# ctxnn/GenConViT

Hardware: AMD Instinct MI355X
Metric: frames/sec (224x224, ed+vae forward) (higher is better)
Workload: dtype f16

## Files before the change

genconvit_amd/_lib.py:

```python
from __future__ import annotations

import ctypes
import ctypes.util
import json
import os
import threading

_HERE = os.path.dirname(os.path.abspath(__file__))
LIB_PATH = os.environ.get("GCV_LIB_PATH") or os.path.join(_HERE, "lib", "libgenconvit_hip.so")

GCV_F32, GCV_BF16, GCV_F16 = 0, 1, 2
ACT_NONE, ACT_RELU, ACT_GELU, ACT_LEAKY = 0, 1, 2, 3
A_PLAIN, A_IM2COL3_POOL, A_IM2COL3_S2 = 0, 1, 2
EPI_BIAS_ACT, EPI_RESID, EPI_POOL4, EPI_CONVT, EPI_SPLITK = 0, 1, 2, 3, 4

c_void_p, c_int, c_int64, c_float, c_char_p, c_size_t = (ctypes.c_void_p, ctypes.c_int, ctypes.c_int64,
                                                         ctypes.c_float, ctypes.c_char_p, ctypes.c_size_t)


class TensorDesc(ctypes.Structure):
    _fields_ = [("name", c_char_p), ("data", c_void_p), ("numel", c_int64), ("on_device", c_int)]


class GemmArgs(ctypes.Structure):
# ... 40 lines not shown
                                c_int, c_void_p, c_void_p]),
    "gcv_vote_segments": (c_int, [c_void_p, c_int, c_int, c_void_p, c_int, c_void_p, c_void_p]),
    "gcv_tap_set": (c_int, [c_void_p, c_char_p, c_void_p, c_size_t]),
    "gcv_tap_clear": (c_int, [c_void_p]),
    "gcv_tap_written": (c_int, [c_void_p, c_char_p]),
    "gcv_profile_enable": (c_int, [c_void_p, c_int]),
    "gcv_profile_report": (c_char_p, [c_void_p]),
    "gcv_k_gemm": (c_int, [c_int, c_int, c_int, ctypes.POINTER(GemmArgs), c_void_p]),
    "gcv_k_stem_ln": (c_int, [c_int, c_void_p, c_int64, c_int64, c_int64, c_int64, c_void_p, c_void_p, c_void_p,
                              c_void_p, c_void_p, c_int, c_int, c_int, c_float, c_void_p]),
    "gcv_k_stem_ln_c": (c_int, [c_int, c_void_p, c_int64, c_int64, c_int64, c_int64, c_void_p, c_void_p, c_void_p,
                                c_void_p, c_void_p, c_int, c_int, c_int, c_int, c_float, c_void_p]),
    "gcv_k_dwconv7_ln": (c_int, [c_int, c_void_p, c_void_p, c_void_p, c_void_p, c_void_p, c_void_p, c_int, c_int,
                                 c_int, c_int, c_float, c_void_p]),
    "gcv_dw_plan": (c_int, [c_int, c_int, c_int, c_int, c_int, c_int, c_void_p]),
    "gcv_convnext_res_ok": (c_int, [c_int, c_int]),
    "gcv_k_ln_patchify": (c_int, [c_int, c_void_p, c_void_p, c_void_p, c_void_p, c_int, c_int, c_int, c_int, c_float,
                                  c_void_p]),
    "gcv_k_layernorm_rows": (c_int, [c_int, c_void_p, c_void_p, c_void_p, c_void_p, c_int64, c_int, c_float, c_void_p]),
    "gcv_k_pool_ln": (c_int, [c_int, c_void_p, c_void_p, c_void_p, c_void_p, c_int, c_int, c_int, c_float, c_void_p]),
    "gcv_k_conv3_first": (c_int, [c_int, c_void_p, c_int64, c_int64, c_int64, c_int64, c_void_p, c_void_p, c_void_p,
                                  c_int, c_int, c_int, c_int, c_int, c_void_p]),
    "gcv_k_convt2_small": (c_int, [c_int, c_void_p, c_void_p, c_void_p, c_void_p, c_int, c_int, c_int, c_int, c_void_p]),
    "gcv_k_reparam": (c_int, [c_int, c_void_p, c_int, c_void_p, c_void_p, c_void_p, c_void_p, c_int, c_int, c_void_p]),
    "gcv_k_head_tail": (c_int, [c_int, c_void_p, c_void_p, c_void_p, c_void_p, c_int, c_int, c_void_p]),
    "gcv_k_head_tail_splitk": (c_int, [c_int, c_void_p, c_int, c_void_p, c_int, c_void_p, c_void_p, c_void_p, c_int, c_int,
                                       c_void_p]),
    "gcv_k_resize_mse": (c_int, [c_int, c_void_p, c_void_p, c_void_p, c_void_p, c_void_p, c_int, c_void_p]),
    "gcv_k_swin_window_attn": (c_int, [c_int, c_void_p, c_void_p, c_void_p, c_int, c_int, c_int, c_int, c_int, c_int,
                                       c_void_p]),
    "gcv_k_patch_merge_ln": (c_int, [c_int, c_void_p, c_void_p, c_void_p, c_void_p, c_int, c_int, c_int, c_int, c_float,
                                     c_void_p]),
    "gcv_k_mean_tokens": (c_int, [c_int, c_void_p, c_void_p, c_int, c_int, c_int, c_void_p]),
    "gcv_k_fused_mlp": (c_int, [c_int, c_int, c_void_p, c_void_p, c_void_p, c_void_p, c_void_p, c_void_p, c_void_p,
                                c_void_p, c_int, c_void_p]),
    "gcv_k_fused_mlp_lnp": (c_int, [c_int, c_int, c_void_p, c_void_p, c_void_p, c_void_p, c_void_p, c_void_p, c_void_p,
                                    c_void_p, c_void_p, c_float, c_int, c_void_p, c_void_p, c_void_p, c_void_p, c_void_p,
                                    c_int, c_void_p]),
    "gcv_k_fused_mlp_timed": (c_int, [c_int, c_int, c_void_p, c_void_p, c_void_p, c_void_p, c_void_p, c_void_p,
                                      c_void_p, c_void_p, c_int, c_int, c_void_p, c_void_p]),
}

_lib = None
_lock = threading.Lock()


# ... 493 lines not shown
```

genconvit_amd/csrc/api.hip:

```cpp
#include "../../include/genconvit_hip.h"

#include <dlfcn.h>

#include <cstdio>
#include <cstdlib>
#include <cstring>
#include <map>
#include <mutex>
#include <set>
#include <sstream>
#include <vector>

#include "cnx_mlp.h"
#include "gemm.h"
#include "kernels.h"
#include "net.h"

namespace gcv {
static thread_local std::string g_err;
void set_error(const std::string& msg) { g_err = msg; }
const char* get_error() { return g_err.c_str(); }

int ensure_dynamic_lds(const void* fn, int bytes) {
  static std::mutex mu;
  static std::map<std::pair<const void*, int>, int> done;
  int dev = 0;
  GCV_CHECK_HIP(hipGetDevice(&dev));
  std::lock_guard<std::mutex> lk(mu);
  auto it = done.find({fn, dev});
  if (it != done.end() && it->second >= bytes) return 0;
  GCV_CHECK_HIP(hipFuncSetAttribute(fn, hipFuncAttributeMaxDynamicSharedMemorySize, bytes));
  done[{fn, dev}] = bytes;
  return 0;
}

hipEvent_t Profiler::get_event() {
// ... 594 lines not shown
}

int gcv_k_layernorm_rows(int dtype, const void* x, const float* w, const float* b, void* out, int64_t rows, int C,
                         float eps, gcv_stream s) {
  DISPATCH_DT(dtype, launch_layernorm_rows<T>((const T*)x, w, b, (T*)out, rows, C, eps, (hipStream_t)s));
}

int gcv_k_pool_ln(int dtype, const void* x, const float* w, const float* b, void* out, int nimg, int HW, int C,
                  float eps, gcv_stream s) {
  DISPATCH_DT(dtype, launch_pool_ln<T>((const T*)x, w, b, (T*)out, nimg, HW, C, eps, (hipStream_t)s));
}

int gcv_k_conv3_first(int dtype, const void* x, int64_t sb, int64_t sc, int64_t sy, int64_t sx, const float* wp,
                      const float* bias, void* out, int nimg, int H, int W, int pool, int act, gcv_stream s) {
  DISPATCH_DT(dtype, launch_conv3_first<T>((const T*)x, sb, sc, sy, sx, wp, bias, (T*)out, nimg, H, W, pool != 0, act,
                                           (hipStream_t)s));
}

int gcv_k_convt2_small(int dtype, const void* x, const float* wp, const float* bias, void* out, int nimg, int H,
                       int W, int act, gcv_stream s) {
  DISPATCH_DT(dtype, launch_convt2_small<T>((const T*)x, wp, bias, (T*)out, nimg, H, W, act, (hipStream_t)s));
}

int gcv_k_reparam(int dtype, const float* partial, int splitk, const float* bias, const float* eps, float* mu_out,
                  void* z_nhwc, int B, int N, gcv_stream s) {
  DISPATCH_DT(dtype, launch_reparam<T>(partial, splitk, bias, eps, mu_out, (T*)z_nhwc, B, N, (hipStream_t)s));
}

int gcv_k_head_tail(int dtype, const void* h, const float* w, const float* bias, float* logits, int B, int K,
                    gcv_stream s) {
  DISPATCH_DT(dtype, launch_head_tail<T>((const T*)h, w, bias, logits, B, K, (hipStream_t)s));
}

int gcv_k_head_tail_splitk(int dtype, const float* partial, int splitk, const float* b1, int act, const float* w,
                           const float* bias, float* logits, int B, int K, gcv_stream s) {
  DISPATCH_DT(dtype, launch_head_tail_splitk<T>(partial, splitk, b1, act, w, bias, logits, B, K, (hipStream_t)s));
}

int gcv_k_resize_mse(int dtype, const void* xhat, const void* img, void* recon, float* msepart, float* mse, int B,
                     gcv_stream s) {
  DISPATCH_DT(dtype, launch_resize_mse<T>((const T*)xhat, (const T*)img, (T*)recon, msepart, mse, B, (hipStream_t)s));
}

int gcv_k_swin_window_attn(int dtype, const void* qkv, const float* rpb, void* out, int nimg, int H, int W, int C,
                           int nH, int shift, gcv_stream s) {
  DISPATCH_DT(dtype, launch_swin_window_attn<T>((const T*)qkv, rpb, (T*)out, nimg, H, W, C, nH, shift, (hipStream_t)s));
// ... 61 lines not shown
```

genconvit_amd/csrc/kern_bf16.hip:

```cpp
#include "kernels_impl.h"
namespace gcv { GCV_INSTANTIATE_KERNELS(bf16_t) }
```

genconvit_amd/csrc/kern_f16.hip:

```cpp
#include "kernels_impl.h"
namespace gcv { GCV_INSTANTIATE_KERNELS(half_t) }
```

genconvit_amd/csrc/net_impl.h:

```cpp
#pragma once
#include <algorithm>
#include <cmath>
#include <cstdlib>
#include <cstring>

#include "cam.h"
#include "cam_bwd.h"
#include "cnx_mlp.h"
#include "gemm.h"
#include "kernels.h"
#include "net.h"
#include "swin.h"

namespace gcv {

template <typename T> inline T host_cvt(float v);
template <> inline float host_cvt<float>(float v) { return v; }
template <> inline half_t host_cvt<half_t>(float v) { return (half_t)v; }
template <> inline bf16_t host_cvt<bf16_t>(float v) {
  uint32_t u;
  std::memcpy(&u, &v, 4);
  uint16_t h;
  if ((u & 0x7fffffffu) > 0x7f800000u) h = (uint16_t)((u >> 16) | 0x40);
  else h = (uint16_t)((u + 0x7fffu + ((u >> 16) & 1u)) >> 16);
  bf16_t r;
  std::memcpy(&r, &h, 2);
  return r;
}

struct WeightStore {
  std::vector<void*> ptrs;
// ... 60 lines not shown
  CnxMlpW<T> mlp;
};
template <typename T> struct CnxW {
  float *stem_w, *stem_b, *stem_lnw, *stem_lnb;
  CnxBlockW<T> blk[kMaxCnxBlocks];
  struct { float *ln_w, *ln_b, *b; T* w; } down[3];
  float *head_lnw, *head_lnb, *head_fc_b;
  T* head_fc_w;
  T *bwd_w1t[3], *bwd_w2t[3], *bwd_downt;
};
template <typename T> struct HeadW {
  T* fc_w;
  float* fc_b;
  float* fc2_w;
  float* fc2_b;
};
template <typename T> struct EdW {
  float *enc1_w, *enc1_b;
  T* enc_w[4];
  float* enc_b[4];
  T* dec_w[4];
  float* dec_b[4];
  float *dec5_w, *dec5_b;
  HeadW<T> head;
};
template <typename T> struct VaeW {
  float *enc1_w, *enc1_b;
  T* enc_w[3];
  float* enc_b[3];
  T *mu_w, *var_w;
  float *mu_b, *var_b;
  T* dec_w[3];
  float* dec_b[3];
  float *dec4_w, *dec4_b;
  HeadW<T> head;
};

template <typename T> struct Stage3In {
  const T* s2 = nullptr;
  const T* x[3] = {nullptr, nullptr, nullptr};
};
template <typename T> struct Seg {
  const T* x;
  int64_t sb, sc, sy, sx;
  int n, H, W;
  T* out;
  int out_ld;
  int act;
  T* pre = nullptr;
  const T** s3 = nullptr;
  Stage3In<T>* in3 = nullptr;
};

template <typename T> struct NetImpl : NetBase {
  WeightStore ws_ed, ws_vae, ws_swin;
  CnxW<T> bb_ed{}, bb_vae{};
  EdW<T> ed{};
// ... 191 lines not shown
  int up_convt_gemm(const TensorMap& w, const std::string& name, int cin, int cout, WeightStore& st, T*& dst) {
    std::vector<float> v;
    GCV_TRY(fetch(w, name, (int64_t)cin * cout * 4, v));
    std::vector<T> o((size_t)cin * cout * 4);
    for (int ci = 0; ci < cin; ++ci)
      for (int co = 0; co < cout; ++co)
        for (int dy = 0; dy < 2; ++dy)
          for (int dx = 0; dx < 2; ++dx)
            o[((size_t)(dy * 2 + dx) * cout + co) * cin + ci] = host_cvt<T>(v[(((size_t)ci * cout + co) * 2 + dy) * 2 + dx]);
    GCV_UP(dst, st, o);
    return 0;
  }
  int up_convt_small(const TensorMap& w, const std::string& name, WeightStore& st, float*& dst) {
    std::vector<float> v;
    GCV_TRY(fetch(w, name, 16 * 3 * 4, v));
    std::vector<float> o(16 * 12);
    for (int ci = 0; ci < 16; ++ci)
      for (int co = 0; co < 3; ++co)
        for (int dy = 0; dy < 2; ++dy)
          for (int dx = 0; dx < 2; ++dx) o[ci * 12 + (dy * 2 + dx) * 3 + co] = v[((ci * 3 + co) * 2 + dy) * 2 + dx];
    GCV_UP(dst, st, o);
    return 0;
  }
  int up_conv_first(const TensorMap& w, const std::string& name, const std::vector<float>* scale, WeightStore& st,
                    float*& dst) {
    std::vector<float> v;
    GCV_TRY(fetch(w, name, 16 * 27, v));
    std::vector<float> o(27 * 16);
    for (int co = 0; co < 16; ++co)
      for (int ci = 0; ci < 3; ++ci)
        for (int ky = 0; ky < 3; ++ky)
          for (int kx = 0; kx < 3; ++kx)
            o[((ky * 3 + kx) * 3 + ci) * 16 + co] = v[((co * 3 + ci) * 3 + ky) * 3 + kx] * (scale ? (*scale)[co] : 1.0f);
    GCV_UP(dst, st, o);
    return 0;
  }

  int pack_mlp(const TensorMap& w, const std::string& fc2_name, int C, WeightStore& st, CnxMlpW<T>& mw) {
    if (mw.kind == MlpKind::Gemm) return 0;
    struct DevBuf {
      float* p = nullptr;
      ~DevBuf() { if (p) (void)hipFree(p); }
    } w2f;
    if (mlp_packs_from_f32(mw.kind)) {
      std::vector<float> v;
      GCV_TRY(fetch(w, fc2_name, (int64_t)4 * C * C, v));
// ... 76 lines not shown

  int load_ed(const TensorMap& w) override {
    GCV_CHECK_HIP(hipSetDevice(device));
    has_ed = false;
    ws_ed.clear();
    GCV_TRY(up_conv_first(w, "encoder.features.0.weight", nullptr, ws_ed, ed.enc1_w));
    GCV_TRY(up_f32(w, "encoder.features.0.bias", 16, ws_ed, ed.enc1_b));
    const int ech[5] = {16, 32, 64, 128, 256};
    const int eidx[4] = {3, 6, 9, 12};
    for (int l = 0; l < 4; ++l) {
      const std::string n = "encoder.features." + std::to_string(eidx[l]);
      GCV_TRY(up_conv_gemm(w, n + ".weight", ech[l + 1], ech[l], 3, 3, nullptr, ws_ed, ed.enc_w[l]));
      GCV_TRY(up_f32(w, n + ".bias", ech[l + 1], ws_ed, ed.enc_b[l]));
    }
    const int dch[5] = {256, 128, 64, 32, 16};
    const int didx[4] = {0, 2, 4, 6};
    for (int l = 0; l < 4; ++l) {
      const std::string n = "decoder.features." + std::to_string(didx[l]);
      GCV_TRY(up_convt_gemm(w, n + ".weight", dch[l], dch[l + 1], ws_ed, ed.dec_w[l]));
      GCV_TRY(up_f32(w, n + ".bias", dch[l + 1], ws_ed, ed.dec_b[l]));
    }
    GCV_TRY(up_convt_small(w, "decoder.features.8.weight", ws_ed, ed.dec5_w));
    GCV_TRY(up_f32(w, "decoder.features.8.bias", 3, ws_ed, ed.dec5_b));
    GCV_TRY(pack_convnext(w, "backbone.", ws_ed, bb_ed));
    GCV_TRY(pack_head(w, ws_ed, ed.head));
    has_ed = true;
    return 0;
  }

  int pack_mu(const TensorMap& w, const std::string& name, T*& dst) {
    auto it = w.find(name);
    const int64_t total = (int64_t)12544 * 25088;
    if (it == w.end() || it->second.numel != total) { set_error("missing or mis-sized '" + name + "'"); return -4; }
    dst = (T*)ws_vae.raw((size_t)total * sizeof(T));
    if (!dst) { set_error("hipMalloc failed for " + name); return -5; }
    const float* src = it->second.data;
    if (it->second.on_device) {
      hipLaunchKernelGGL((pack_mu_kernel<T>), dim3((unsigned)cdiv64(total, 256)), dim3(256), 0, 0, src, dst, total);
      GCV_CHECK_HIP(hipGetLastError());
      GCV_CHECK_HIP(hipDeviceSynchronize());
      return 0;
    }
    constexpr int64_t kRows = 512;
    struct DevBuf {
      float* p = nullptr;
      ~DevBuf() { if (p) (void)hipFree(p); }
// ... 35 lines not shown
        GCV_UP(vae.enc1_b, ws_vae, bias);
      } else {
        GCV_TRY(up_conv_gemm(w, cn + ".weight", c, ech[l], 3, 3, &scale, ws_vae, vae.enc_w[l - 1]));
        GCV_UP(vae.enc_b[l - 1], ws_vae, bias);
      }
    }
    GCV_TRY(pack_mu(w, "encoder.mu.weight", vae.mu_w));
    GCV_TRY(up_f32(w, "encoder.mu.bias", 12544, ws_vae, vae.mu_b));
    vae.var_w = nullptr;
    vae.var_b = nullptr;
    if (w.count("encoder.var.weight")) {
      GCV_TRY(pack_mu(w, "encoder.var.weight", vae.var_w));
      GCV_TRY(up_f32(w, "encoder.var.bias", 12544, ws_vae, vae.var_b));
    }
    const int dch[4] = {256, 64, 32, 16};
    const int didx[3] = {0, 2, 4};
    for (int l = 0; l < 3; ++l) {
      const std::string n = "decoder.features." + std::to_string(didx[l]);
      GCV_TRY(up_convt_gemm(w, n + ".weight", dch[l], dch[l + 1], ws_vae, vae.dec_w[l]));
      GCV_TRY(up_f32(w, n + ".bias", dch[l + 1], ws_vae, vae.dec_b[l]));
    }
    GCV_TRY(up_convt_small(w, "decoder.features.6.weight", ws_vae, vae.dec4_w));
    GCV_TRY(up_f32(w, "decoder.features.6.bias", 3, ws_vae, vae.dec4_b));
    GCV_TRY(pack_convnext(w, "convnext_backbone.", ws_vae, bb_vae));
    GCV_TRY(pack_head(w, ws_vae, vae.head));
    has_vae = true;
    return 0;
  }

  int load_swin(const TensorMap& w, const std::string& prefix) override {
    GCV_CHECK_HIP(hipSetDevice(device));
    has_swin = false;
    ws_swin.clear();
    GCV_TRY((pack_swin<T>(*this, w, prefix, swin)));
    has_swin = true;
    return 0;
  }

  int run_convnext(const CnxW<T>& w, const Seg<T>* segs, int nseg, bool keep = false, const TapPass* tp = nullptr) {
    int segn[4], h[4], wd[4];
    int64_t m[4], moff[4], M = 0;
    int ntot = 0;
    GCV_REQUIRE(nseg >= 1 && nseg <= 4, "1..4 segments");
    for (int s = 0; s < nseg; ++s) {
      GCV_REQUIRE(segs[s].H % 4 == 0 && segs[s].W % 4 == 0 && segs[s].n > 0, "segment geometry");
      segn[s] = segs[s].n;
// ... 314 lines not shown
    T* rec = arena.get<T>((int64_t)B * 224 * 224 * 3);
    T* feat = arena.get<T>((int64_t)B * 2000);
    T* bbpre = ex ? arena.get<T>((int64_t)B * 2000) : nullptr;
    if (!arena.dry && arena.overflow) { set_error("workspace arena too small"); return -6; }

    GCV_TRY(run("ed.enc1_conv3_relu_pool", 2.0 * B * 224 * 224 * 16 * 27,
                sizeof(T) * (double)B * (3 * 224 * 224 + 16 * 112 * 112), [&] {
      return launch_conv3_first<T>(x, 3 * 224 * 224, 224 * 224, 224, 1, ed.enc1_w, ed.enc1_b, e1, B, 224, 224, true,
                                   ACT_RELU, cur);
    }));
    {
      const T* in[4] = {e1, e2, e3, e4};
      T* out[4] = {e2, e3, e4, e5};
      const int Hs[4] = {112, 56, 28, 14};
      const int cl[4] = {4, 5, 6, 7};
      for (int l = 0; l < 4; ++l) {
        GemmArgs g{};
        g.A = in[l]; g.Wt = ed.enc_w[l]; g.C = out[l]; g.bias = ed.enc_b[l];
        g.M = B * Hs[l] * Hs[l]; g.N = 2 << cl[l]; g.K = 9 << cl[l]; g.ldc = g.N; g.act = ACT_RELU; g.splitk = 1;
        g.H = Hs[l]; g.W = Hs[l]; g.cin_log2 = cl[l];
        GCV_TRY(gemm("ed.enc_conv3_relu_pool", g, A_IM2COL3_POOL, EPI_POOL4));
      }
    }
    {
      const T* in[4] = {e5, d1, d2, d3};
      T* out[4] = {d1, d2, d3, d4};
      const int Hs[4] = {7, 14, 28, 56};
      const int col[4] = {7, 6, 5, 4};
      for (int l = 0; l < 4; ++l) {
        GemmArgs g{};
        g.A = in[l]; g.lda = 2 << col[l]; g.Wt = ed.dec_w[l]; g.C = out[l]; g.bias = ed.dec_b[l];
        g.M = B * Hs[l] * Hs[l]; g.N = 4 << col[l]; g.K = 2 << col[l]; g.act = ACT_RELU; g.splitk = 1;
        g.H = Hs[l]; g.W = Hs[l]; g.cout_log2 = col[l];
        GCV_TRY(gemm("ed.dec_convT_relu", g, A_PLAIN, EPI_CONVT));
      }
    }
    GCV_TRY(run("ed.dec5_convT_relu", 2.0 * B * 112 * 112 * 16 * 12,
                sizeof(T) * (double)B * (16 * 112 * 112 + 3 * 224 * 224),
                [&] { return launch_convt2_small<T>(d4, ed.dec5_w, ed.dec5_b, rec, B, 112, 112, ACT_RELU, cur); }));
    Seg<T> segs[2];
    segs[0] = Seg<T>{rec, (int64_t)224 * 224 * 3, 1, 224 * 3, 3, B, 224, 224, feat, 2000, ACT_GELU};
    segs[1] = Seg<T>{x, (int64_t)3 * 224 * 224, 224 * 224, 224, 1, B, 224, 224, feat + 1000, 2000, ACT_GELU};
    const T* s3[2] = {nullptr, nullptr};
    Stage3In<T> in3[2];
    const float* head_part = nullptr;
    if (ex)
      for (int q = 0; q < 2; ++q) {
        segs[q].pre = bbpre + 1000 * q; segs[q].s3 = &s3[q];
        if (ex->layer == 2) segs[q].in3 = &in3[q];
      }
    const TapPass tp{"ed", 2, 0, {B, B}, {224, 224}, {224, 224}};
    GCV_TRY(run_convnext(bb_ed, segs, 2, false, taps.empty() ? nullptr : &tp));
    GCV_TRY(run_head(ed.head, feat, B, ACT_GELU, logits, ex ? &head_part : nullptr));
    if (ex) {
      const int hwp[2] = {49, 49}, side[2] = {7, 7}, off[2] = {0, 49}, side2[2] = {14, 14};
      GCV_TRY(explain_tail(bb_ed, ed.head, ACT_GELU, B, head_part, bbpre, logits, s3, hwp, side, off, 1, *ex, in3, side2, "ed"));
    }
    if (!taps.empty()) {
      const T* et[5] = {e1, e2, e3, e4, e5};
      const int64_t ee[5] = {112 * 112 * 16, 56 * 56 * 32, 28 * 28 * 64, 14 * 14 * 128, 7 * 7 * 256};
      const T* dt[4] = {d1, d2, d3, d4};
      const int64_t de[4] = {14 * 14 * 128, 28 * 28 * 64, 56 * 56 * 32, 112 * 112 * 16};
// ... 74 lines not shown
      for (int l = 0; l < 3; ++l) {
        GemmArgs g{};
        g.A = in[l]; g.Wt = vae.enc_w[l]; g.C = out[l]; g.bias = vae.enc_b[l];
        g.M = B * (Hs[l] / 2) * (Hs[l] / 2); g.N = 2 << cl[l]; g.K = 9 << cl[l]; g.ldc = g.N; g.act = ACT_LEAKY;
        g.splitk = 1; g.H = Hs[l]; g.W = Hs[l]; g.cin_log2 = cl[l];
        GCV_TRY(gemm("vae.enc_conv3s2_bn_leaky", g, A_IM2COL3_S2, EPI_BIAS_ACT));
      }
    }
    {
      GemmArgs g{};
      g.A = v4; g.lda = 25088; g.Wt = vae.mu_w; g.partial = part; g.M = B; g.N = 12544; g.K = 25088;
      g.splitk = SPLITK; g.k_per_split = KPS; g.act = ACT_NONE;
      GCV_TRY(gemm("vae.mu_gemm_splitk", g, A_PLAIN, EPI_SPLITK));
      GCV_TRY(run("vae.reparam", 4.0 * B * 12544, 4.0 * (SPLITK + 2) * (double)B * 12544, [&] {
        return launch_reparam<T>(part, SPLITK, vae.mu_b, eps, mu, z, B, 12544, cur);
      }));
      if (kl) {
        g.Wt = vae.var_w;
        GCV_TRY(gemm("vae.var_gemm_splitk", g, A_PLAIN, EPI_SPLITK));
        GCV_TRY(run("vae.kl", 6.0 * B * 12544, 4.0 * (SPLITK + 1) * (double)B * 12544,
                    [&] { return launch_kl(part, SPLITK, vae.var_b, mu, rowsum, kl, B, 12544, cur); }));
      }
    }
    {
      const T* in[3] = {z, d1, d2};
      T* out[3] = {d1, d2, d3};
      const int Hs[3] = {7, 14, 28};
      const int cin[3] = {256, 64, 32};
      const int col[3] = {6, 5, 4};
      for (int l = 0; l < 3; ++l) {
        GemmArgs g{};
        g.A = in[l]; g.lda = cin[l]; g.Wt = vae.dec_w[l]; g.C = out[l]; g.bias = vae.dec_b[l];
        g.M = B * Hs[l] * Hs[l]; g.N = 4 << col[l]; g.K = cin[l]; g.act = ACT_LEAKY; g.splitk = 1;
        g.H = Hs[l]; g.W = Hs[l]; g.cout_log2 = col[l];
        GCV_TRY(gemm("vae.dec_convT_leaky", g, A_PLAIN, EPI_CONVT));
      }
    }
    GCV_TRY(run("vae.dec4_convT_leaky", 2.0 * B * 56 * 56 * 16 * 12,
                sizeof(T) * (double)B * (16 * 56 * 56 + 3 * 112 * 112),
                [&] { return launch_convt2_small<T>(d3, vae.dec4_w, vae.dec4_b, xhat, B, 56, 56, ACT_LEAKY, cur); }));
    if (after_chain && !arena.dry) GCV_TRY(after_chain());
    if (split) { GCV_TRY(run_convnext(bb_vae, &segs[1], 1, true, tapping ? &tp1 : nullptr)); }
    else { GCV_TRY(run_convnext(bb_vae, segs, 2, false, tapping ? &tp0 : nullptr)); }
    join.now();
    if (tapping) {
      const T* vt[4] = {v1, v2, v3, v4};
      const int64_t ve[4] = {112 * 112 * 16, 56 * 56 * 32, 28 * 28 * 64, 14 * 14 * 128};
      const T* dt[3] = {d1, d2, d3};
      const int64_t de[3] = {14 * 14 * 64, 28 * 28 * 32, 56 * 56 * 16};
      for (int l = 0; l < 4; ++l) GCV_TRY(tap_net(("vae.v" + std::to_string(l + 1)).c_str(), vt[l], B * ve[l] * sizeof(T)));
      GCV_TRY(tap_net("vae.mu", mu, (size_t)B * 12544 * sizeof(float)));
      GCV_TRY(tap_net("vae.z", z, (size_t)B * 12544 * sizeof(T)));
      for (int l = 0; l < 3; ++l) GCV_TRY(tap_net(("vae.d" + std::to_string(l + 1)).c_str(), dt[l], B * de[l] * sizeof(T)));
      GCV_TRY(tap_net("vae.xhat", xhat, (size_t)B * 112 * 112 * 3 * sizeof(T)));
      GCV_TRY(tap_net("vae.feat", feat, (size_t)B * 2000 * sizeof(T)));
    }
    GCV_TRY(run_head(vae.head, feat, B, ACT_RELU, logits, ex ? &head_part : nullptr));
    if (ex) {
      const int hwp[2] = {49, 9}, side[2] = {7, 3}, off[2] = {0, 49}, side2[2] = {14, 7};
      GCV_TRY(explain_tail(bb_vae, vae.head, ACT_RELU, B, head_part, bbpre, logits, s3, hwp, side, off, 0, *ex, in3, side2, "vae"));
    }
    if (recon224 || mse) {
      GCV_TRY(run("vae.resize_mse", 30.0 * B * 224 * 224, sizeof(T) * (double)B * (3 * 112 * 112 + 6 * 224 * 224), [&] {
// ... 53 lines not shown
```

include/genconvit_hip.h:

```cpp
#ifndef GENCONVIT_HIP_H
#define GENCONVIT_HIP_H

#include <stddef.h>
#include <stdint.h>

#ifdef __cplusplus
extern "C" {
#endif

#if defined(GCV_BUILD)
#pragma GCC visibility push(default)
#endif

typedef struct gcv_handle gcv_handle;
typedef void* gcv_stream;

enum { GCV_F32 = 0, GCV_BF16 = 1, GCV_F16 = 2 };
enum { GCV_CONVNEXT_TINY = 0, GCV_CONVNEXT_LARGE = 1 };
enum { GCV_LARGE_MAX_BATCH = 256 };
enum { GCV_ACT_NONE = 0, GCV_ACT_RELU = 1, GCV_ACT_GELU = 2, GCV_ACT_LEAKY = 3 };

typedef struct {
  const char* name;
  const void* data;
// ... 80 lines not shown
} gcv_gemm_args;

int gcv_k_gemm(int dtype, int a_mode, int epi, const gcv_gemm_args* a, gcv_stream s);
int gcv_k_stem_ln(int dtype, const void* x, int64_t sb, int64_t sc, int64_t sy, int64_t sx, const float* wp,
                  const float* bias, const float* lnw, const float* lnb, void* out, int nimg, int Ho, int Wo,
                  float eps, gcv_stream s);
int gcv_k_stem_ln_c(int dtype, const void* x, int64_t sb, int64_t sc, int64_t sy, int64_t sx, const float* wp,
                    const float* bias, const float* lnw, const float* lnb, void* out, int nimg, int Ho, int Wo, int C,
                    float eps, gcv_stream s);
int gcv_k_dwconv7_ln(int dtype, const void* x, const float* wdw, const float* bdw, const float* lnw,
                     const float* lnb, void* y, int nimg, int H, int W, int C, float eps, gcv_stream s);
int gcv_dw_plan(int dtype, int nimg, int H, int W, int C, int aligned, int* out5);
int gcv_convnext_res_ok(int arch, int res);
int gcv_k_ln_patchify(int dtype, const void* x, const float* w, const float* b, void* out, int nimg, int H, int W,
                      int C, float eps, gcv_stream s);
int gcv_k_layernorm_rows(int dtype, const void* x, const float* w, const float* b, void* out, int64_t rows, int C,
                         float eps, gcv_stream s);
int gcv_k_pool_ln(int dtype, const void* x, const float* w, const float* b, void* out, int nimg, int HW, int C,
                  float eps, gcv_stream s);
int gcv_k_conv3_first(int dtype, const void* x, int64_t sb, int64_t sc, int64_t sy, int64_t sx, const float* wp,
                      const float* bias, void* out, int nimg, int H, int W, int pool, int act, gcv_stream s);
int gcv_k_convt2_small(int dtype, const void* x, const float* wp, const float* bias, void* out, int nimg, int H,
                       int W, int act, gcv_stream s);
int gcv_k_reparam(int dtype, const float* partial, int splitk, const float* bias, const float* eps, float* mu_out,
                  void* z_nhwc, int B, int N, gcv_stream s);
int gcv_k_head_tail(int dtype, const void* h, const float* w, const float* bias, float* logits, int B, int K,
                    gcv_stream s);
int gcv_k_head_tail_splitk(int dtype, const float* partial, int splitk, const float* b1, int act, const float* w,
                           const float* bias, float* logits, int B, int K, gcv_stream s);
int gcv_k_resize_mse(int dtype, const void* xhat, const void* img, void* recon, float* msepart, float* mse, int B,
                     gcv_stream s);

int gcv_k_swin_window_attn(int dtype, const void* qkv, const float* rpb, void* out, int nimg, int H, int W, int C,
                           int nH, int shift, gcv_stream s);
int gcv_k_patch_merge_ln(int dtype, const void* x, const float* w, const float* b, void* out, int nimg, int H, int W,
                         int C, float eps, gcv_stream s);
int gcv_k_mean_tokens(int dtype, const void* x, void* out, int nimg, int L, int C, gcv_stream s);

int gcv_k_fused_mlp(int dtype, int C, const void* x, const void* w1, const float* b1, const float* w2_f32,
                    const float* b2, const float* gamma, const void* resid, void* out, int M, gcv_stream s);
int gcv_k_fused_mlp_lnp(int dtype, int C, const void* x, const void* w1, const float* b1, const float* w2_f32,
                        const float* b2, const float* gamma, const void* resid, const float* ln_w, const float* ln_b,
                        float eps, int nseg, const int* tok0, const int* hw, const int* wd, const int* out0, void* out, int M,
                        gcv_stream s);
int gcv_k_fused_mlp_timed(int dtype, int C, const void* x, const void* w1, const float* b1, const float* w2_f32,
                          const float* b2, const float* gamma, const void* resid, void* out, int M, int iters,
// ... 11 lines not shown
```

Baseline: 18890.

## Fuse ED and VAE transposed-conv decoder chains into one LDS-resident kernel

Adds a single kernel that runs all 2x2-stride transposed-conv decoder layers plus the final small conv for each 8-pixel latent tile. Intermediates stay in shared memory, so the per-layer global round trips and separate launches go away. Layers use MFMA with weights pre-packed into fragment order at load time, and the next layer's first weight fragment is prefetched. In exchange it needs large LDS per block (two workgroups per CU) and grid parallelism is limited to B*49/8 blocks, so work per block may serialize. The fused path applies only to 16-bit types when no taps are requested.

```diff
diff --git a/genconvit_amd/_lib.py b/genconvit_amd/_lib.py
--- a/genconvit_amd/_lib.py
+++ b/genconvit_amd/_lib.py
@@ -86,6 +86,8 @@
     "gcv_k_conv3_first": (c_int, [c_int, c_void_p, c_int64, c_int64, c_int64, c_int64, c_void_p, c_void_p, c_void_p,
                                   c_int, c_int, c_int, c_int, c_int, c_void_p]),
     "gcv_k_convt2_small": (c_int, [c_int, c_void_p, c_void_p, c_void_p, c_void_p, c_int, c_int, c_int, c_int, c_void_p]),
+    "gcv_k_convt_pack": (c_int, [c_int, c_void_p, c_int, c_int, c_void_p, c_void_p]),
+    "gcv_k_decoder_fused": (c_int, [c_int, c_int, c_void_p, c_void_p, c_void_p, c_void_p, c_void_p, c_void_p, c_int, c_void_p]),
     "gcv_k_reparam": (c_int, [c_int, c_void_p, c_int, c_void_p, c_void_p, c_void_p, c_void_p, c_int, c_int, c_void_p]),
     "gcv_k_head_tail": (c_int, [c_int, c_void_p, c_void_p, c_void_p, c_void_p, c_int, c_int, c_void_p]),
     "gcv_k_head_tail_splitk": (c_int, [c_int, c_void_p, c_int, c_void_p, c_int, c_void_p, c_void_p, c_void_p, c_int, c_int,
diff --git a/genconvit_amd/csrc/api.hip b/genconvit_amd/csrc/api.hip
--- a/genconvit_amd/csrc/api.hip
+++ b/genconvit_amd/csrc/api.hip
@@ -12,6 +12,7 @@
 #include <vector>
 
 #include "cnx_mlp.h"
+#include "decoder_fused.h"
 #include "gemm.h"
 #include "kernels.h"
 #include "net.h"
@@ -652,6 +653,27 @@
   DISPATCH_DT(dtype, launch_convt2_small<T>((const T*)x, wp, bias, (T*)out, nimg, H, W, act, (hipStream_t)s));
 }
 
+int gcv_k_convt_pack(int dtype, const void* wt, int N, int K, void* dst, gcv_stream s) {
+  switch (dtype) {
+    case GCV_BF16: return launch_convt_pack<bf16_t>((const bf16_t*)wt, N, K, (bf16_t*)dst, (hipStream_t)s);
+    case GCV_F16:  return launch_convt_pack<half_t>((const half_t*)wt, N, K, (half_t*)dst, (hipStream_t)s);
+    default: set_error("convt_pack: 16-bit storage only"); return -2;
+  }
+}
+
+int gcv_k_decoder_fused(int dtype, int kind, const void* x, const void* wpk, const float* const* bias, const float* w5,
+                        const float* b5, void* out, int npix, gcv_stream s) {
+  GCV_REQUIRE(bias, "null bias list");
+  DecoderArgs a{};
+  a.x = x; a.wpk = wpk; a.w5 = w5; a.b5 = b5; a.out = out; a.npix = npix;
+  for (int l = 0; l < (kind == DEC_ED ? 4 : 3); ++l) a.bias[l] = bias[l];
+  switch (dtype) {
+    case GCV_BF16: return launch_decoder_fused<bf16_t>(kind, a, (hipStream_t)s);
+    case GCV_F16:  return launch_decoder_fused<half_t>(kind, a, (hipStream_t)s);
+    default: set_error("decoder_fused: 16-bit storage only"); return -2;
+  }
+}
+
 int gcv_k_reparam(int dtype, const float* partial, int splitk, const float* bias, const float* eps, float* mu_out,
                   void* z_nhwc, int B, int N, gcv_stream s) {
   DISPATCH_DT(dtype, launch_reparam<T>(partial, splitk, bias, eps, mu_out, (T*)z_nhwc, B, N, (hipStream_t)s));
diff --git a/genconvit_amd/csrc/decoder_fused.h b/genconvit_amd/csrc/decoder_fused.h
--- /dev/null
+++ b/genconvit_amd/csrc/decoder_fused.h
@@ -0,0 +1,302 @@
+#pragma once
+#include "common.h"
+#include "gemm.h"
+
+namespace gcv {
+
+enum { DEC_ED = 0, DEC_VAE = 1 };
+
+struct DecoderArgs {
+  const void* x;
+  const void* wpk;
+  const float* bias[4];
+  const float* w5;
+  const float* b5;
+  void* out;
+  int npix;
+};
+
+inline int64_t decoder_packed_elems(int kind) {
+  return kind == DEC_ED ? 4 * (256 * 128 + 128 * 64 + 64 * 32 + 32 * 16) : 4 * (256 * 64 + 64 * 32 + 32 * 16);
+}
+template <typename T> int launch_convt_pack(const T* wt, int N, int K, T* dst, hipStream_t s);
+template <typename T> int launch_decoder_fused(int kind, const DecoderArgs& a, hipStream_t s);
+
+#ifdef GCV_DECODER_FUSED_IMPL
+
+template <int C1, int NL> struct DecShape {
+  static constexpr int P = 8;
+  static constexpr int cin(int l) { return l == 0 ? 256 : C1 >> (l - 1); }
+  static constexpr int cout(int l) { return C1 >> l; }
+  static constexpr int ntok(int l) { return P << (2 * l); }
+  static constexpr int stride(int l) { return cin(l) * 2 + 16; }
+  static constexpr int kChunkTok = ntok(NL - 1) < 256 ? ntok(NL - 1) : 256;
+  static constexpr int kChunkPlane = kChunkTok * 32 + 64;
+  static constexpr int kChunkBytes = 4 * kChunkPlane;
+  static constexpr int kLastTok = 4 * kChunkTok / 256;
+  static constexpr int region(int r) {
+    int m = (NL & 1) == r ? kChunkBytes : 0;
+    for (int l = 0; l < NL; ++l)
+      if ((l & 1) == r && ntok(l) * stride(l) > m) m = ntok(l) * stride(l);
+    return m;
+  }
+  static constexpr int woff(int l) {
+    int o = 0;
+    for (int i = 0; i < l; ++i) o += 4 * cout(i) * cin(i);
+    return o;
+  }
+  static constexpr int boff(int l) {
+    int o = 0;
+    for (int i = 0; i < l; ++i) o += cout(i);
+    return o;
+  }
+  static constexpr int kBiasFloats = 256;
+  static constexpr int lds = region(0) + region(1) + 16 * 12 * 4 + kBiasFloats * 4;
+  static_assert(cout(NL - 1) == 16, "the last layer reads 16 channels");
+  static_assert(ntok(NL - 1) % kChunkTok == 0 && boff(NL) <= 252, "whole chunks; room for the biases");
+};
+
+template <int KS> struct WFrag { u32x4 w[KS]; };
+template <typename T, int KS>
+__device__ __forceinline__ void load_wfrag(const T* __restrict__ wpk, int nb, int lane, WFrag<KS>& f) {
+  const u32x4* wp = reinterpret_cast<const u32x4*>(wpk) + (int64_t)nb * KS * 64 + lane;
+#pragma unroll
+  for (int ks = 0; ks < KS; ++ks) f.w[ks] = wp[ks * 64];
+}
+
+template <typename T, int K, int COUT, int ACT, int TB, int G, int VALID, int DSTR, int DQSTR, class Prefetch>
+__device__ __forceinline__ void convt_mfma_layer(const unsigned char* src, unsigned char* dst, const T* __restrict__ wpk,
+                                                 const float* sbias, int wave, int lane, WFrag<K / 16>& cur,
+                                                 Prefetch&& prefetch) {
+  constexpr int NB = 4 * COUT / 32, KS = K / 16, SSTR = K * 2 + 16, ITEMS = NB * (TB / G), NIT = ITEMS / 4;
+  static_assert(TB % G == 0 && (VALID == TB * 32 || (TB == 1 && (VALID & (VALID - 1)) == 0)), "token blocks");
+  static_assert(ITEMS % 4 == 0, "the same number of items for every wave");
+  typedef T t4 __attribute__((ext_vector_type(4)));
+  const int lr = lane & 31, lh = lane >> 5;
+#pragma unroll
+  for (int i = 0; i < NIT; ++i) {
+    const int it = wave + 4 * i;
+    const int nb = it % NB, tg = it / NB;
+    WFrag<KS> nxt;
+    if (i + 1 < NIT) load_wfrag<T, KS>(wpk, (it + 4) % NB, lane, nxt);
+    else prefetch();
+    f32x16 acc[G];
+    int m[G];
+    const unsigned char* sp[G];
+#pragma unroll
+    for (int g = 0; g < G; ++g) {
+#pragma unroll
+      for (int r = 0; r < 16; ++r) acc[g][r] = 0.0f;
+      m[g] = (tg * G + g) * 32 + lr;
+      sp[g] = src + (VALID < 32 ? (m[g] & (VALID - 1)) : m[g]) * SSTR + lh * 16;
+    }
+#pragma unroll
+    for (int ks = 0; ks < KS; ++ks) {
+#pragma unroll
+      for (int g = 0; g < G; ++g) Mfma<T>::run(cur.w[ks], *reinterpret_cast<const u32x4*>(sp[g] + ks * 32), acc[g]);
+    }
+#pragma unroll
+    for (int q = 0; q < 4; ++q) {
+      const int n = nb * 32 + 8 * q + 4 * lh;
+      const int co = n & (COUT - 1), dq = n / COUT;
+      const f32x4 bv = *reinterpret_cast<const f32x4*>(sbias + co);
+#pragma unroll
+      for (int g = 0; g < G; ++g) {
+        if (VALID < 32 && m[g] >= VALID) continue;
+        float v[4];
+#pragma unroll
+        for (int e = 0; e < 4; ++e) v[e] = act_fn<ACT>(acc[g][4 * q + e] + bv[e]);
+        const t4 o = {from_f<T>(v[0]), from_f<T>(v[1]), from_f<T>(v[2]), from_f<T>(v[3])};
+        *reinterpret_cast<t4*>(dst + (DQSTR ? dq * DQSTR + m[g] * DSTR : (m[g] * 4 + dq) * DSTR) + co * 2) = o;
+      }
+    }
+    if (i + 1 < NIT) cur = nxt;
+  }
+}
+
+template <typename T, int NL, int ACT, int TPT, int PLANE>
+__device__ __forceinline__ void convt_last(const unsigned char* chunk, const float* sW, const float* sb5,
+                                           T* __restrict__ out, int pix0, int npix, int tid) {
+  constexpr int SIDE = 1 << NL, TPP = SIDE * SIDE, S = 2 * SIDE, HW = 7 * S;
+  const float b3[3] = {sb5[0], sb5[1], sb5[2]};
+  u32x4 lo[TPT], hi[TPT];
+  float acc[TPT][12];
+  int gp[TPT], yy[TPT], xx[TPT];
+#pragma unroll
+  for (int j = 0; j < TPT; ++j) {
+    const int idx = tid + 256 * j;
+    const int pl = idx / TPP, rem = idx % TPP, y = rem / SIDE, x = rem % SIDE;
+    gp[j] = pix0 + pl; yy[j] = y; xx[j] = x;
+    int t = 0;
+#pragma unroll
+    for (int b = NL - 1; b >= 0; --b) t = t * 4 + ((y >> b) & 1) * 2 + ((x >> b) & 1);
+    const int tl = pl * TPP + t;
+    const unsigned char* src = chunk + (tl & 3) * PLANE + (tl >> 2) * 32;
+    lo[j] = *reinterpret_cast<const u32x4*>(src);
+    hi[j] = *reinterpret_cast<const u32x4*>(src + 16);
+#pragma unroll
+    for (int k = 0; k < 12; ++k) acc[j][k] = b3[k % 3];
+  }
+#pragma unroll 1
+  for (int h = 0; h < 4; ++h) {
+    float v[TPT][4];
+#pragma unroll
+    for (int j = 0; j < TPT; ++j) {
+      const uint32_t d0 = h == 0 ? lo[j][0] : (h == 1 ? lo[j][2] : (h == 2 ? hi[j][0] : hi[j][2]));
+      const uint32_t d1 = h == 0 ? lo[j][1] : (h == 1 ? lo[j][3] : (h == 2 ? hi[j][1] : hi[j][3]));
+      v[j][0] = to_f(__builtin_bit_cast(T, (unsigned short)(d0 & 0xffffu)));
+      v[j][1] = to_f(__builtin_bit_cast(T, (unsigned short)(d0 >> 16)));
+      v[j][2] = to_f(__builtin_bit_cast(T, (unsigned short)(d1 & 0xffffu)));
+      v[j][3] = to_f(__builtin_bit_cast(T, (unsigned short)(d1 >> 16)));
+    }
+#pragma unroll
+    for (int c4 = 0; c4 < 4; ++c4) {
+      const float4* wr = reinterpret_cast<const float4*>(sW + (4 * h + c4) * 12);
+#pragma unroll
+      for (int g4 = 0; g4 < 3; ++g4) {
+        const float4 w4 = wr[g4];
+#pragma unroll
+        for (int j = 0; j < TPT; ++j) {
+          acc[j][4 * g4] = fmaf(v[j][c4], w4.x, acc[j][4 * g4]);
+          acc[j][4 * g4 + 1] = fmaf(v[j][c4], w4.y, acc[j][4 * g4 + 1]);
+          acc[j][4 * g4 + 2] = fmaf(v[j][c4], w4.z, acc[j][4 * g4 + 2]);
+          acc[j][4 * g4 + 3] = fmaf(v[j][c4], w4.w, acc[j][4 * g4 + 3]);
+        }
+      }
+    }
+  }
+#pragma unroll
+  for (int j = 0; j < TPT; ++j) {
+    if (gp[j] >= npix) continue;
+    const int b = gp[j] / 49, hw = gp[j] - b * 49, py = hw / 7, px = hw - py * 7;
+#pragma unroll
+    for (int dy = 0; dy < 2; ++dy) {
+      T* o = out + (((int64_t)b * HW + py * S + 2 * yy[j] + dy) * HW + px * S + 2 * xx[j]) * 3;
+      uint32_t pk[3];
+#pragma unroll
+      for (int k = 0; k < 3; ++k) {
+        const T e0 = from_f<T>(apply_act(acc[j][dy * 6 + 2 * k], ACT)), e1 = from_f<T>(apply_act(acc[j][dy * 6 + 2 * k + 1], ACT));
+        pk[k] = (uint32_t)__builtin_bit_cast(unsigned short, e0) | ((uint32_t)__builtin_bit_cast(unsigned short, e1) << 16);
+      }
+      typedef uint32_t u32x3 __attribute__((ext_vector_type(3)));
+      *reinterpret_cast<u32x3*>(o) = u32x3{pk[0], pk[1], pk[2]};
+    }
+  }
+}
+
+template <int NB, int TB> constexpr int dec_group() {
+  constexpr int g0 = NB * TB / 4 < 1 ? 1 : NB * TB / 4, g1 = g0 < TB ? g0 : TB;
+  return g1 < 4 ? g1 : 4;
+}
+
+template <typename T, int C1, int NL, int ACT, int L>
+__device__ __forceinline__ void decoder_layers(unsigned char* r0, unsigned char* r1, const float* sW, const float* sB,
+                                               const DecoderArgs& a, int pix0, int tid,
+                                               WFrag<DecShape<C1, NL>::cin(L) / 16>& cur) {
+  using S = DecShape<C1, NL>;
+  const int wave = tid >> 6, lane = tid & 63;
+  unsigned char* src = (L & 1) ? r1 : r0;
+  unsigned char* dst = (L & 1) ? r0 : r1;
+  const T* wpk = (const T*)a.wpk + S::woff(L);
+  constexpr int K = S::cin(L), COUT = S::cout(L), NB = 4 * COUT / 32;
+  if constexpr (L < NL - 1) {
+    constexpr int TOK = S::ntok(L), TB = (TOK + 31) / 32, G = dec_group<NB, TB>();
+    constexpr int KS1 = S::cin(L + 1) / 16, NB1 = 4 * S::cout(L + 1) / 32;
+    WFrag<KS1> first;
+    convt_mfma_layer<T, K, COUT, ACT, TB, G, TOK, S::stride(L + 1), 0>(src, dst, wpk, sB + S::boff(L), wave, lane, cur, [&] {
+      load_wfrag<T, KS1>((const T*)a.wpk + S::woff(L + 1), wave % NB1, lane, first);
+    });
+    __syncthreads();
+    decoder_layers<T, C1, NL, ACT, L + 1>(r0, r1, sW, sB, a, pix0, tid, first);
+  } else {
+    constexpr int CT = S::kChunkTok, NCH = S::ntok(L) / CT, TB = CT / 32, G = dec_group<NB, TB>(), TPP = 1 << (2 * NL);
+#pragma unroll 1
+    for (int c = 0; c < NCH; ++c) {
+      convt_mfma_layer<T, K, COUT, ACT, TB, G, CT, 32, S::kChunkPlane>(src + c * CT * S::stride(L), dst, wpk, sB + S::boff(L), wave, lane, cur, [] {});
+      __syncthreads();
+      convt_last<T, NL, ACT, S::kLastTok, S::kChunkPlane>(dst, sW, sB + 252, (T*)a.out, pix0 + c * (4 * CT / TPP), a.npix, tid);
+      __syncthreads();
+    }
+  }
+}
+
+template <typename T, int C1, int NL, int ACT>
+__global__ void __launch_bounds__(256, 2) decoder_fused_kernel(const DecoderArgs a) {
+  using S = DecShape<C1, NL>;
+  extern __shared__ __attribute__((aligned(16))) unsigned char smem[];
+  unsigned char* r0 = smem;
+  unsigned char* r1 = smem + S::region(0);
+  float* sW = reinterpret_cast<float*>(smem + S::region(0) + S::region(1));
+  float* sB = sW + 16 * 12;
+  const int tid = threadIdx.x;
+  const int pix0 = blockIdx.x * S::P;
+  WFrag<16> first;
+  load_wfrag<T, 16>((const T*)a.wpk, (tid >> 6) % (4 * S::cout(0) / 32), tid & 63, first);
+  if (tid < 16 * 12) sW[tid] = a.w5[tid];
+  {
+    int l = 0, o = tid;
+#pragma unroll
+    for (int i = 0; i < NL - 1; ++i)
+      if (tid >= S::boff(i + 1)) { l = i + 1; o = tid - S::boff(i + 1); }
+    if (tid < S::boff(NL)) sB[tid] = a.bias[l][o];
+    if (tid >= 252 && tid < 255) sB[tid] = a.b5[tid - 252];
+  }
+  {
+    static_assert(S::P * 32 == 256, "one piece per thread");
+    const int tok = tid >> 5, c = tid & 31;
+    u32x4 v = {0u, 0u, 0u, 0u};
+    if (pix0 + tok < a.npix) v = *reinterpret_cast<const u32x4*>((const T*)a.x + (int64_t)(pix0 + tok) * 256 + c * 8);
+    *reinterpret_cast<u32x4*>(r0 + tok * S::stride(0) + c * 16) = v;
+  }
+  __syncthreads();
+  decoder_layers<T, C1, NL, ACT, 0>(r0, r1, sW, sB, a, pix0, tid, first);
+}
+
+template <typename T>
+__global__ void __launch_bounds__(256) convt_pack_kernel(const T* __restrict__ wt, T* __restrict__ dst, int N, int K) {
+  const int ci = blockIdx.x * 256 + threadIdx.x;
+  if (ci >= N * K / 8) return;
+  const int lane = ci & 63, blk = ci >> 6, KS = K / 16;
+  const int nb = blk / KS, ks = blk - nb * KS;
+  const int n = nb * 32 + (lane & 31), k = ks * 16 + 8 * (lane >> 5);
+  *reinterpret_cast<u32x4*>(dst + (int64_t)ci * 8) = *reinterpret_cast<const u32x4*>(wt + (int64_t)n * K + k);
+}
+
+template <typename T> int launch_convt_pack(const T* wt, int N, int K, T* dst, hipStream_t s) {
+  GCV_REQUIRE(wt && dst && N > 0 && K > 0 && N % 32 == 0 && K % 16 == 0, "convt_pack: N % 32 == 0 and K % 16 == 0");
+  GCV_REQUIRE(((reinterpret_cast<uintptr_t>(wt) | reinterpret_cast<uintptr_t>(dst)) & 15u) == 0, "convt_pack: 16-byte aligned");
+  hipLaunchKernelGGL((convt_pack_kernel<T>), dim3(cdiv(N * K / 8, 256)), dim3(256), 0, s, wt, dst, N, K);
+  GCV_CHECK_HIP(hipGetLastError());
+  return 0;
+}
+
+template <typename T> int launch_decoder_fused(int kind, const DecoderArgs& a, hipStream_t s) {
+  static_assert(sizeof(T) == 2, "the fused decoders are built for 16-bit storage");
+  GCV_REQUIRE(kind == DEC_ED || kind == DEC_VAE, "decoder_fused: kind is DEC_ED or DEC_VAE");
+  GCV_REQUIRE(a.x && a.wpk && a.w5 && a.b5 && a.out && a.npix > 0 && a.npix % 49 == 0, "decoder_fused: npix = B * 49");
+  const int nl = kind == DEC_ED ? 4 : 3;
+  for (int l = 0; l < nl; ++l) GCV_REQUIRE(a.bias[l] && (reinterpret_cast<uintptr_t>(a.bias[l]) & 15u) == 0, "decoder_fused: bias");
+  GCV_REQUIRE(((reinterpret_cast<uintptr_t>(a.x) | reinterpret_cast<uintptr_t>(a.wpk)) & 15u) == 0 &&
+                  (reinterpret_cast<uintptr_t>(a.out) & 3u) == 0, "decoder_fused: alignment");
+  const int grid = cdiv(a.npix, 8);
+  if (kind == DEC_ED) {
+    using S = DecShape<128, 4>;
+    static_assert(2 * S::lds <= 160 * 1024, "two workgroups per CU");
+    auto kernel = decoder_fused_kernel<T, 128, 4, ACT_RELU>;
+    GCV_ENSURE_LDS(kernel, S::lds);
+    hipLaunchKernelGGL(kernel, dim3(grid), dim3(256), S::lds, s, a);
+  } else {
+    using S = DecShape<64, 3>;
+    hipLaunchKernelGGL((decoder_fused_kernel<T, 64, 3, ACT_LEAKY>), dim3(grid), dim3(256), S::lds, s, a);
+  }
+  GCV_CHECK_HIP(hipGetLastError());
+  return 0;
+}
+
+#define GCV_INSTANTIATE_DECODER_FUSED(T)                                          \
+  template int launch_convt_pack<T>(const T*, int, int, T*, hipStream_t);         \
+  template int launch_decoder_fused<T>(int, const DecoderArgs&, hipStream_t);
+
+#endif
+
+}
diff --git a/genconvit_amd/csrc/kern_bf16.hip b/genconvit_amd/csrc/kern_bf16.hip
--- a/genconvit_amd/csrc/kern_bf16.hip
+++ b/genconvit_amd/csrc/kern_bf16.hip
@@ -1,2 +1,4 @@
+#define GCV_DECODER_FUSED_IMPL
+#include "decoder_fused.h"
 #include "kernels_impl.h"
-namespace gcv { GCV_INSTANTIATE_KERNELS(bf16_t) }
+namespace gcv { GCV_INSTANTIATE_KERNELS(bf16_t) GCV_INSTANTIATE_DECODER_FUSED(bf16_t) }
diff --git a/genconvit_amd/csrc/kern_f16.hip b/genconvit_amd/csrc/kern_f16.hip
--- a/genconvit_amd/csrc/kern_f16.hip
+++ b/genconvit_amd/csrc/kern_f16.hip
@@ -1,2 +1,4 @@
+#define GCV_DECODER_FUSED_IMPL
+#include "decoder_fused.h"
 #include "kernels_impl.h"
-namespace gcv { GCV_INSTANTIATE_KERNELS(half_t) }
+namespace gcv { GCV_INSTANTIATE_KERNELS(half_t) GCV_INSTANTIATE_DECODER_FUSED(half_t) }
diff --git a/genconvit_amd/csrc/net_impl.h b/genconvit_amd/csrc/net_impl.h
--- a/genconvit_amd/csrc/net_impl.h
+++ b/genconvit_amd/csrc/net_impl.h
@@ -7,6 +7,7 @@
 #include "cam.h"
 #include "cam_bwd.h"
 #include "cnx_mlp.h"
+#include "decoder_fused.h"
 #include "gemm.h"
 #include "kernels.h"
 #include "net.h"
@@ -113,6 +114,7 @@
   T* dec_w[4];
   float* dec_b[4];
   float *dec5_w, *dec5_b;
+  T* dec_pk;
   HeadW<T> head;
 };
 template <typename T> struct VaeW {
@@ -124,6 +126,7 @@
   T* dec_w[3];
   float* dec_b[3];
   float *dec4_w, *dec4_b;
+  T* dec_pk;
   HeadW<T> head;
 };
 
@@ -361,6 +364,20 @@
     GCV_UP(dst, st, o);
     return 0;
   }
+  int pack_decoder(int kind, T* const* dec_w, const int* ch, int nl, WeightStore& st, T*& dst) {
+    dst = nullptr;
+    if constexpr (sizeof(T) == 2) {
+      dst = (T*)st.raw((size_t)decoder_packed_elems(kind) * sizeof(T));
+      if (!dst) { set_error("hipMalloc failed for the packed decoder weights"); return -5; }
+      int64_t off = 0;
+      for (int l = 0; l < nl; ++l) {
+        GCV_TRY(launch_convt_pack<T>(dec_w[l], 4 * ch[l + 1], ch[l], dst + off, nullptr));
+        off += (int64_t)4 * ch[l + 1] * ch[l];
+      }
+      GCV_CHECK_HIP(hipDeviceSynchronize());
+    }
+    return 0;
+  }
   int up_conv_first(const TensorMap& w, const std::string& name, const std::vector<float>* scale, WeightStore& st,
                     float*& dst) {
     std::vector<float> v;
@@ -483,6 +500,7 @@
     }
     GCV_TRY(up_convt_small(w, "decoder.features.8.weight", ws_ed, ed.dec5_w));
     GCV_TRY(up_f32(w, "decoder.features.8.bias", 3, ws_ed, ed.dec5_b));
+    GCV_TRY(pack_decoder(DEC_ED, ed.dec_w, dch, 4, ws_ed, ed.dec_pk));
     GCV_TRY(pack_convnext(w, "backbone.", ws_ed, bb_ed));
     GCV_TRY(pack_head(w, ws_ed, ed.head));
     has_ed = true;
@@ -564,6 +582,7 @@
     }
     GCV_TRY(up_convt_small(w, "decoder.features.6.weight", ws_vae, vae.dec4_w));
     GCV_TRY(up_f32(w, "decoder.features.6.bias", 3, ws_vae, vae.dec4_b));
+    GCV_TRY(pack_decoder(DEC_VAE, vae.dec_w, dch, 3, ws_vae, vae.dec_pk));
     GCV_TRY(pack_convnext(w, "convnext_backbone.", ws_vae, bb_vae));
     GCV_TRY(pack_head(w, ws_vae, vae.head));
     has_vae = true;
@@ -924,7 +943,16 @@
         GCV_TRY(gemm("ed.enc_conv3_relu_pool", g, A_IM2COL3_POOL, EPI_POOL4));
       }
     }
-    {
+    if (sizeof(T) == 2 && taps.empty()) {
+      GCV_TRY(run("ed.dec_fused_convT_relu", 2.0 * B * 49 * (4 * 131072.0 + 256 * 16 * 12),
+                  sizeof(T) * (double)B * (256 * 49 + 3 * 224 * 224), [&] {
+        if constexpr (sizeof(T) == 2) {
+          DecoderArgs a{e5, ed.dec_pk, {ed.dec_b[0], ed.dec_b[1], ed.dec_b[2], ed.dec_b[3]}, ed.dec5_w, ed.dec5_b, rec, B * 49};
+          return launch_decoder_fused<T>(DEC_ED, a, cur);
+        }
+        return 0;
+      }));
+    } else {
       const T* in[4] = {e5, d1, d2, d3};
       T* out[4] = {d1, d2, d3, d4};
       const int Hs[4] = {7, 14, 28, 56};
@@ -936,10 +964,10 @@
         g.H = Hs[l]; g.W = Hs[l]; g.cout_log2 = col[l];
         GCV_TRY(gemm("ed.dec_convT_relu", g, A_PLAIN, EPI_CONVT));
       }
-    }
-    GCV_TRY(run("ed.dec5_convT_relu", 2.0 * B * 112 * 112 * 16 * 12,
-                sizeof(T) * (double)B * (16 * 112 * 112 + 3 * 224 * 224),
-                [&] { return launch_convt2_small<T>(d4, ed.dec5_w, ed.dec5_b, rec, B, 112, 112, ACT_RELU, cur); }));
+      GCV_TRY(run("ed.dec5_convT_relu", 2.0 * B * 112 * 112 * 16 * 12,
+                  sizeof(T) * (double)B * (16 * 112 * 112 + 3 * 224 * 224),
+                  [&] { return launch_convt2_small<T>(d4, ed.dec5_w, ed.dec5_b, rec, B, 112, 112, ACT_RELU, cur); }));
+    }
     Seg<T> segs[2];
     segs[0] = Seg<T>{rec, (int64_t)224 * 224 * 3, 1, 224 * 3, 3, B, 224, 224, feat, 2000, ACT_GELU};
     segs[1] = Seg<T>{x, (int64_t)3 * 224 * 224, 224 * 224, 224, 1, B, 224, 224, feat + 1000, 2000, ACT_GELU};
@@ -1060,7 +1088,16 @@
                     [&] { return launch_kl(part, SPLITK, vae.var_b, mu, rowsum, kl, B, 12544, cur); }));
       }
     }
-    {
+    if (sizeof(T) == 2 && taps.empty()) {
+      GCV_TRY(run("vae.dec_fused_convT_leaky", 2.0 * B * 49 * (3 * 65536.0 + 64 * 16 * 12),
+                  sizeof(T) * (double)B * (256 * 49 + 3 * 112 * 112), [&] {
+        if constexpr (sizeof(T) == 2) {
+          DecoderArgs a{z, vae.dec_pk, {vae.dec_b[0], vae.dec_b[1], vae.dec_b[2], nullptr}, vae.dec4_w, vae.dec4_b, xhat, B * 49};
+          return launch_decoder_fused<T>(DEC_VAE, a, cur);
+        }
+        return 0;
+      }));
+    } else {
       const T* in[3] = {z, d1, d2};
       T* out[3] = {d1, d2, d3};
       const int Hs[3] = {7, 14, 28};
@@ -1073,10 +1110,10 @@
         g.H = Hs[l]; g.W = Hs[l]; g.cout_log2 = col[l];
         GCV_TRY(gemm("vae.dec_convT_leaky", g, A_PLAIN, EPI_CONVT));
       }
-    }
-    GCV_TRY(run("vae.dec4_convT_leaky", 2.0 * B * 56 * 56 * 16 * 12,
-                sizeof(T) * (double)B * (16 * 56 * 56 + 3 * 112 * 112),
-                [&] { return launch_convt2_small<T>(d3, vae.dec4_w, vae.dec4_b, xhat, B, 56, 56, ACT_LEAKY, cur); }));
+      GCV_TRY(run("vae.dec4_convT_leaky", 2.0 * B * 56 * 56 * 16 * 12,
+                  sizeof(T) * (double)B * (16 * 56 * 56 + 3 * 112 * 112),
+                  [&] { return launch_convt2_small<T>(d3, vae.dec4_w, vae.dec4_b, xhat, B, 56, 56, ACT_LEAKY, cur); }));
+    }
     if (after_chain && !arena.dry) GCV_TRY(after_chain());
     if (split) { GCV_TRY(run_convnext(bb_vae, &segs[1], 1, true, tapping ? &tp1 : nullptr)); }
     else { GCV_TRY(run_convnext(bb_vae, segs, 2, false, tapping ? &tp0 : nullptr)); }
diff --git a/include/genconvit_hip.h b/include/genconvit_hip.h
--- a/include/genconvit_hip.h
+++ b/include/genconvit_hip.h
@@ -126,6 +126,9 @@
                       const float* bias, void* out, int nimg, int H, int W, int pool, int act, gcv_stream s);
 int gcv_k_convt2_small(int dtype, const void* x, const float* wp, const float* bias, void* out, int nimg, int H,
                        int W, int act, gcv_stream s);
+int gcv_k_convt_pack(int dtype, const void* wt, int N, int K, void* dst, gcv_stream s);
+int gcv_k_decoder_fused(int dtype, int kind, const void* x, const void* wpk, const float* const* bias, const float* w5,
+                        const float* b5, void* out, int npix, gcv_stream s);
 int gcv_k_reparam(int dtype, const float* partial, int splitk, const float* bias, const float* eps, float* mu_out,
                   void* z_nhwc, int B, int N, gcv_stream s);
 int gcv_k_head_tail(int dtype, const void* h, const float* w, const float* bias, float* logits, int B, int K,
```

New measurement: 18910 (median of 2 runs). No clear change (+0.1%).
